# mkeeter/fidget

Measured on AMD Instinct MI355X. Metric: Mvoxel/s (interval+point eval) on prospero.vm 1024^3, higher is better.
Workload: dtype f32; 1 GPU; prospero.vm 3D heightmap+normals 1024^3, HipShape render hints (the library's tiles: 128/32/8, or 32/8 when the root level has few tiles), world_to_model=I

## Files before the change

### fidget_amd/csrc/capi_render.hpp

```cpp
static fhip_status bind_inputs(fhip_ctx* ctx, const fhip_tape* tape, const int32_t* axis_slots, const uint64_t* keys,
                               const float* vals, uint32_t n, FhRender& P) {
    const fh::HostTape& t = tape->t;
    std::vector<char> bound(FH_MAX_INPUTS, 0);
    for (uint32_t s = 0; s < FH_MAX_INPUTS; s++) { P.in_kind[s] = 3; P.in_value[s] = 0.0f; }
    for (int a = 0; a < 3; a++) {
        const int s = axis_slots ? axis_slots[a] : t.vars.axis[a];
        if (s >= 0 && s < FH_MAX_INPUTS) { P.in_kind[s] = (uint32_t)a; bound[s] = 1; }
    }
    for (uint32_t i = 0; i < n; i++) {
        const int s = axis_slots ? (int)keys[i] : t.vars.slot_of(3, keys[i]);
        if (s >= 0 && s < FH_MAX_INPUTS) { P.in_value[s] = vals[i]; bound[s] = 1; }
    }
    for (uint32_t s = 0; s < t.n_vars; s++)
        if (!bound[s]) return fail(ctx, FHIP_ERR_MISSING_VAR, "a variable of the shape has no value");
    return FHIP_OK;
}

struct HostSpans {
    double t[8] = {0, 0, 0, 0, 0, 0, 0, 0};
    uint64_t n = 0;
    std::chrono::steady_clock::time_point last;
    void start() { last = std::chrono::steady_clock::now(); }
    void mark(int k) { const auto now = std::chrono::steady_clock::now(); t[k] += std::chrono::duration<double, std::micro>(now - last).count(); last = now; }
    void frame() {
// ... 227 lines not shown
struct KaPrune1 { FhRenderState* S; uint32_t level, big, max_choices, mode; };
struct KaColumns { FhRenderState* S; uint32_t n_waves, slots, depmask, flags, pad[2]; const void* table; uint32_t nfpl, layers; };
struct KaNormals { FhRenderState* S; uint32_t n_waves, slots, z_lo, z_hi, bucket_cap, mode; };

struct FrameStreams { hipStream_t s[N_ROLES]; Role cur; hipStream_t on() const { return s[cur]; } };
static FrameStreams frame_streams(const fhip_ctx* ctx, Role at = CALLER) { return FrameStreams{{ctx->stream, ctx->stream_pre, ctx->stream2, ctx->stream3}, at}; }
static hipError_t hop(FrameStreams& fs, Role to, hipEvent_t ev) {
    if (to == fs.cur) return hipSuccess;
    const hipError_t e = hipEventRecord(ev, fs.on());
    fs.cur = to;
    return e != hipSuccess ? e : hipStreamWaitEvent(fs.on(), ev, 0);
}
static ScheduleInputs schedule_inputs(const fhip_ctx* ctx, int out_is_device) {
    ScheduleInputs in;
    in.no_tiles_v = ctx->opt.no_tiles_v; in.no_zrep = ctx->opt.no_zrep; in.column_walk = ctx->opt.column_walk; in.column_group = ctx->opt.column_group;
    in.frame_pipeline = ctx->frame_pipeline; in.use_pipeline = ctx->use_pipeline; in.profiling = ctx->profiling; in.slab_contexts = ctx->slab_contexts;
    in.has_side = ctx->stream2 != nullptr; in.has_tail = ctx->stream3 != nullptr; in.has_flags = ctx->host_flags != nullptr; in.out_is_device = out_is_device != 0;
    return in;
}
static char* rare_file(const fhip_ctx* ctx, const FhRenderState* dS, uint32_t rare_stride) {
    if (!rare_stride) return nullptr;
    return (char*)ctx->rare_scratch.p + (size_t)(dS - (const FhRenderState*)ctx->state.p) * FH_RARE_BLOCKS * rare_stride;
}
static void tiles_by_groups(fhip_ctx* ctx, const RenderSetup& R, FhRenderState* dS, hipStream_t st) {
    const int gg = blocks_for(ctx, R.lds_tiles_group, 8);
    KaTiles ka = {dS, 0, 1, R.group_regs, R.group_choices, (uint32_t)gg, (ctx->probe ? 1u : 0u) | 2u | 4u | 8u, 0, 0};
    (void)launch_asm(ctx, st, FH_ASM_TILES, (uint32_t)gg, &ka, sizeof(ka), R.lds_tiles_group);
    const uint32_t blocks = R.S.qcap[0], root_words = (R.S.troot_choices + 15) / 16, group_words = (R.group_choices + 15) / 16;
    if (R.S.top_chain && R.S.n_top > 64u * FH_CHAIN_SEG) FH_KLAUNCH(k_tchain3d_chunks, dim3(WAVE, blocks), dim3(WAVE), 0, st, dS);
    else if (R.S.top_chain) FH_KLAUNCH(k_tchain3d, dim3(WAVE, blocks), dim3(WAVE), 0, st, dS);
    else FH_KLAUNCH(k_ttop3d, dim3(blocks), dim3(WAVE), 0, st, dS);
    if (R.classify_only || !root_words) FH_KLAUNCH(k_tmark3d, dim3(blocks), dim3(WAVE), 0, st, dS);
    if (R.classify_only) return;
    if (root_words) FH_KLAUNCH(k_tscatter3d, dim3(root_words + 1, blocks), dim3(WAVE), 0, st, dS, group_words, root_words);
    KaPrune1 kp = {dS, 0, 1, R.S.troot_choices, 2};
    if (!R.prune2) { (void)launch_asm(ctx, st, FH_ASM_PRUNE1, blocks * 64, &kp, sizeof(kp)); return; }
    hipEvent_t ea = nullptr, eb = nullptr;
    if (ctx->profiling) { (void)hipEventCreate(&ea); (void)hipEventCreate(&eb); (void)hipEventRecord(ea, st); }
    FH_KLAUNCH(k_prune2, dim3(blocks * FH_P2_PER_SLOT), dim3(FH_P2_WPB * FH_P2_WPC * 64), R.lds_prune2, st, dS, 0u, 1u, root_words,
                       (const uint2*)R.d_links, (const uint2*)R.d_ctab, 2u, R.S.troot_len, R.S.troot_choices, R.p2_cap_kept,
                       (const uint32_t*)(R.d_ctab + std::max<uint32_t>(R.S.troot_choices, 1)), R.n_chain);
    size_t kp_bytes = sizeof(kp);
    void* extra[] = {HIP_LAUNCH_PARAM_BUFFER_POINTER, &kp, HIP_LAUNCH_PARAM_BUFFER_SIZE, &kp_bytes, HIP_LAUNCH_PARAM_END};
    (void)hipModuleLaunchKernel(ctx->asm_fn[FH_ASM_PRUNE1], blocks * 64, 1, 1, WAVE, 1, 1, 0, st, nullptr, extra);
    if (ctx->profiling) { (void)hipEventRecord(eb, st); ctx->asm_events.push_back({FH_ASM_PRUNE1, {ea, eb}}); }
}
static void tiles_asm(fhip_ctx* ctx, const RenderSetup& R, const LevelPlan& L, FhRenderState* dS, int level, FrameStreams& fs) {
    const int gs = blocks_for(ctx, R.lds_tiles_small, 8), gb = blocks_big(ctx, R, R.lds_tiles_big, 8);
    const int K_TILES = R.asm_tiles_t ? FH_ASM_TILES_T : FH_ASM_TILES;
    auto big_stream = [&] { return L.fork_big ? fs.s[SIDE] : fs.on(); };
    KaTiles ka = {dS, (uint32_t)level, 0, SMALL_REGS, SMALL_CHOICES, (uint32_t)gs, (ctx->probe ? 1u : 0u) | (L.exp ? 2u : 0u), 0, 0};
// ... 39 lines not shown
    if (R.full) FH_KLAUNCH((k_teval3d<true, true>), dim3(gb), dim3(WAVE), R.lds_tiles_big, st, dS, level);
    else FH_KLAUNCH((k_teval3d<false, true>), dim3(gb), dim3(WAVE), R.lds_tiles_big, st, dS, level);
}
static void launch_tiles_mono(fhip_ctx* ctx, const RenderSetup& R, FhRenderState* dS, int level, bool is3d, hipStream_t st) {
    const int gs = blocks_for(ctx, R.lds_tiles_small, 8), gb = blocks_big(ctx, R, R.lds_tiles_big, 8);
    launch(ctx, st, FHIP_K_TILES, [&] {
        if (is3d) { if (R.full) FH_LAUNCH_TILES(true, true, true, gb, R.lds_tiles_big); else FH_LAUNCH_TILES(true, false, true, gb, R.lds_tiles_big); }
        else { if (R.full) FH_LAUNCH_TILES(false, true, true, gb, R.lds_tiles_big); else FH_LAUNCH_TILES(false, false, true, gb, R.lds_tiles_big); }
    });
    if (level > 0)
        launch(ctx, st, FHIP_K_TILES, [&] {
            if (is3d) { if (R.full) FH_LAUNCH_TILES(true, true, false, gs, R.lds_tiles_small); else FH_LAUNCH_TILES(true, false, false, gs, R.lds_tiles_small); }
            else { if (R.full) FH_LAUNCH_TILES(false, true, false, gs, R.lds_tiles_small); else FH_LAUNCH_TILES(false, false, false, gs, R.lds_tiles_small); }
        });
}
static void launch_tiles(fhip_ctx* ctx, const RenderSetup& R, const LevelPlan& L, FhRenderState* dS, int level, bool is3d, FrameStreams& fs) {
    if (L.path == LevelPlan::MONO) return launch_tiles_mono(ctx, R, dS, level, is3d, fs.on());
    const int gp = ctx->n_cu * 8;
    launch(ctx, fs.on(), FHIP_K_TILES, [&] {
        if (is3d) FH_KLAUNCH(k_tsetup3d, dim3(gp), dim3(WAVE), 0, fs.on(), dS, level);
        else FH_KLAUNCH(k_tsetup2d, dim3(gp), dim3(WAVE), 0, fs.on(), dS, level);
    });
    launch(ctx, fs.on(), FHIP_K_TILES, [&] {
        if (L.path == LevelPlan::GROUPS) tiles_by_groups(ctx, R, dS, fs.on());
        else if (L.path == LevelPlan::ASM) tiles_asm(ctx, R, L, dS, level, fs);
        else tiles_hip(ctx, R, dS, level, fs.on());
    });
    const bool last = level + 1 == (int)R.S.P.n_levels;
    const int gpush = last ? ctx->n_cu * L.push_mul : gp;
    launch(ctx, fs.on(), FHIP_K_TILES, [&] {
        const uint32_t rb = L.rare ? FH_RARE_BLOCKS : 0u;
        if (is3d) FH_KLAUNCH(k_tpush3d, dim3(gpush + rb, last ? 1 : 17), dim3(WAVE), 0, fs.on(), dS, level, rb, rare_file(ctx, dS, L.rare_stride), L.rare_stride);
        else {
            if (!R.classify_only) FH_KLAUNCH(k_tpush2d, dim3(gpush), dim3(WAVE), 0, fs.on(), dS, level);
            const uint32_t slots_max = R.S.qcap[level] * ((level == 0 && R.groups) ? R.S.n_tgroups : 1u);
            FH_KLAUNCH(k_tfill2d, dim3(64, slots_max), dim3(256), 0, fs.on(), dS, level);
        }
    });
}

static fhip_status render2d_frame(fhip_ctx* ctx, const fhip_tape* tape, const fhip_render2d_config* cfg, float* out,
                                  int out_is_device) {
    if (ctx->is_cancelled()) return fail(ctx, FHIP_ERR_CANCELLED, "cancelled");
    RenderSetup R;
    memset(&R.S, 0, sizeof(R.S));
    FhRender& P = R.S.P;
    P.width = cfg->width; P.height = cfg->height; P.depth = 0; P.z = cfg->z; P.pixel_perfect = cfg->pixel_perfect ? 1 : 0;
// ... 528 lines not shown
```

### fidget_amd/csrc/frame_schedule.hpp

```cpp
#pragma once
#include <stddef.h>
#include <stdint.h>

#include <algorithm>
#include <vector>

#include "frame_plan.hpp"
#include "render_state.h"

static const uint32_t V32_REGS = 32, V32_CHOICES = 256, V64_REGS = 64, V64_CHOICES = 512;
static const uint32_t FH_RARE_BLOCKS = 8;

enum Role : uint8_t { CALLER = 0, PRE, SIDE, TAIL, N_ROLES };

struct ScheduleInputs {
    int no_tiles_v = 0, no_zrep = 0, column_walk = 1, column_group = 2;
    bool frame_pipeline = true, use_pipeline = true, profiling = false, has_side = true, has_tail = true, has_flags = true;
    uint32_t slab_contexts = 4;
    bool out_is_device = true, huge = false, whole = true;
    bool frames_queued = false;
    uint32_t pre_turn = 0;
    uint32_t rare_seen = 1, last_leaves = 0;
};

struct LevelPlan {
    enum Path : uint8_t { MONO, GROUPS, ASM, HIP } path = MONO;
    Role rest_on = CALLER;
    bool per_slab = false, exp = false;
    bool v32 = false, small_lds = false, v64 = false, both_lists = false;
    bool mid = false, rest = false;
    bool rare = false;
    bool fork_big = false;
    uint32_t rare_stride = 0; int push_mul = 2;
};

struct FrameSchedule {
    bool fpipe = false, lone = false, alt_pre = false, takes_turn = false;
    Role root = CALLER, l1_flags = CALLER, l1 = CALLER, fork_on = CALLER, tiles = CALLER, lists = CALLER, leaf = CALLER, normals = CALLER;
    bool fork_to_side = false, fork_to_tail = false, ev_pre = false, pre_implied = false, aux_edge = false;
    bool coarse = false, pipe = false, tiles_first = false; uint32_t NC = 1;
    int slab_first = 0, slab_stop = 0, n_rendered = 0;
    bool rare = false; uint32_t rare_stride = 0;
    enum LeafWalk : uint8_t { HIP_LEAVES, BY_LIST, BY_COLUMNS, BY_BLOCKS } leaf_walk = HIP_LEAVES;
    bool by_list = false, by_columns = false; uint32_t g = 0;
    uint32_t list_waves = 0, table_words = 0; int reset_blocks = 1;
    bool normals_on = true;
    LevelPlan level[FH_MAX_LEVELS];
};

static bool frame_pipelined(const ScheduleInputs& in) { return in.frame_pipeline && in.use_pipeline && !in.profiling && in.out_is_device && !in.huge; }

static LevelPlan plan_level(const RenderSetup& R, const ScheduleInputs& in, int level, bool is3d, uint32_t rare_stride, Role on, Role rest_on) {
    LevelPlan L;
#ifdef FH_PUSH_MUL
    L.push_mul = FH_PUSH_MUL;
#endif
    L.rare_stride = rare_stride; L.rest_on = rest_on;
    const uint32_t pre = R.S.pre_levels, l = (uint32_t)level;
    const FhRender& P = R.S.P;
    if (!R.split) return L;
    L.per_slab = pre > 0 && l >= pre;
    L.exp = R.prune1 && l < R.exp_levels;
    L.rare = rare_stride && is3d && R.asm_tiles && !in.no_tiles_v && level > 0 && L.per_slab && !L.exp;
    if (R.groups && level == 0) { L.path = LevelPlan::GROUPS; return L; }
    if (!R.asm_tiles) { L.path = LevelPlan::HIP; return L; }
    L.path = LevelPlan::ASM;
    L.fork_big = level > 0 && l < pre && in.use_pipeline && !in.profiling && in.has_side && on == CALLER && is3d;
    const bool vk = !in.no_tiles_v && !L.exp;
    L.both_lists = level > 0 && vk && l < pre && !L.fork_big;
    L.v32 = level > 0 && vk && !L.both_lists; L.small_lds = level > 0 && !vk;
    if (L.rare) return L;
    const bool root_v64 = vk && level == 0 && is3d && P.max_regs <= V64_REGS && P.max_choices <= V64_CHOICES;
    L.v64 = vk && (level > 0 || root_v64);
    L.rest = !L.v64 || P.max_regs > V64_REGS || P.max_choices > V64_CHOICES;
    L.mid = !vk && level > 0 && l < pre && R.lds_tiles_mid * 2 <= R.lds_tiles_big;
    return L;
}

static FrameSchedule schedule_frame(const RenderSetup& R, const ScheduleInputs& in) {
    FrameSchedule F;
    const FhRender& P = R.S.P;
    const uint32_t pre = R.S.pre_levels, n_groups = R.groups_per_slab, slabs = R.slab_hi - R.slab_lo;
    F.fpipe = frame_pipelined(in);
    F.alt_pre = F.fpipe && P.n_levels == 2 && R.column_inv && in.no_zrep == 0 && in.has_tail && in.whole;
    F.lone = F.fpipe && !in.frames_queued;
#ifdef FH_EXP_NO_LONE
    F.lone = false;
#endif
    F.takes_turn = F.fpipe && !F.lone && F.alt_pre;
    F.root = !F.fpipe || F.lone ? CALLER : (F.takes_turn && (in.pre_turn & 1u) ? TAIL : PRE);
    F.coarse = pre && n_groups;
    F.pipe = in.use_pipeline && !in.profiling && slabs > 1 && n_groups > 0 && !R.big_hbm;
    F.NC = F.pipe ? std::min<uint32_t>(in.slab_contexts, slabs) : 1;
    F.slab_first = (int)R.slab_hi - 1; F.slab_stop = (int)R.slab_stop;
    F.n_rendered = n_groups ? std::max(0, F.slab_first - F.slab_stop + 1) : 0;
    const bool l1_side = F.fpipe && !F.lone && pre > 1 && in.has_side && slabs > 1 && n_groups > 0;
    F.tiles_first = F.pipe && l1_side && R.root_invariant && in.has_tail && R.asm_points && slabs <= F.NC;
    F.l1 = l1_side ? SIDE : F.root;
    F.l1_flags = F.tiles_first ? F.root : F.l1;
    const bool tail_to_side = F.fpipe && !F.lone && F.pipe && pre == 1 && in.has_side;
    F.fork_on = F.tiles_first ? TAIL : tail_to_side ? SIDE : F.l1;
    F.tiles = !F.pipe ? CALLER : F.tiles_first ? TAIL : SIDE;
    F.fork_to_side = F.pipe && F.fork_on != SIDE;
    F.fork_to_tail = F.tiles_first;
    F.pre_implied = F.fpipe && F.pipe && pre == 1 && in.has_side && F.fork_on == SIDE;
    F.ev_pre = F.fpipe && F.fork_on != CALLER && !F.pre_implied;
    const bool on_main = F.tiles_first && in.frames_queued;
    F.aux_edge = F.pipe && in.has_tail && R.asm_points && !on_main && !F.alt_pre;
    F.lists = F.normals = F.aux_edge ? TAIL : CALLER;
    const size_t stride = (std::max(std::max(R.lds_tiles_big, R.lds_points_big), R.lds_normals_big) + 255) / 256 * 256;
    F.rare = R.split && R.asm_tiles && R.asm_points && R.asm_normals && !R.big_hbm && in.has_flags && in.rare_seen == 0 &&
             stride * FH_RARE_BLOCKS * 4 <= ((size_t)256 << 20);
    F.rare_stride = F.rare ? (uint32_t)stride : 0u;
    const uint32_t layers = P.slab / 8;
    F.by_list = in.column_walk == 1 && R.column_inv && R.split && R.zrep && R.asm_points && R.asm_normals && layers <= 64 && in.has_flags;
    F.table_words = F.by_list ? 0u : R.table_words;
    F.list_waves = (R.n_footprints + 63) / 64 * 64;
    if (F.by_list && in.last_leaves) F.list_waves = std::min(F.list_waves, (in.last_leaves + in.last_leaves / 8 + 63) / 64 * 64);
    F.reset_blocks = (int)std::max<uint32_t>(1, std::min<uint32_t>(1024, (std::max(F.table_words, n_groups) + 255) / 256));
    F.by_columns = in.column_walk == 2 || ((in.column_walk == 1 || in.column_walk == 3) && R.column_inv);
    const uint32_t g_opt = (uint32_t)std::min(std::max(in.column_group, 0), 6);
    F.g = F.by_columns ? 6u : (R.smooth_tape && g_opt > 1 ? g_opt - 1 : g_opt);
    F.leaf_walk = !R.asm_points ? FrameSchedule::HIP_LEAVES : F.by_list ? FrameSchedule::BY_LIST
// ... 11 lines not shown
```

### fidget_amd/csrc/gen_tilesv.py

```python
from gen_interp import OPS, UNSUPPORTED, HSTRIDE_LOG2
import gen_tiles as GT
from gen_tiles import (Tiles, S_KERNARG, S_STATE, S_LEVEL, S_BIG, S_MAXREGS, S_MAXCH, S_ARENA, S_ARENACAP, S_SLOTS, S_NSLOTS, S_SLOT, S_OFF,
                       S_LEN, S_RC, S_ACT, S_SIGN, S_ABSM, S_DECIDED, S_CI, S_NREGS, S_NCH, S_PRUNE, S_BASE, S_MA, S_MB, S_HBASE, S_TAPE,
                       S_REM, S_K, S_W0, S_W1, S_T0, S_OUT, S_A, S_T1, S_OP, S_RET, S_T64, S_LIVE, S_ALIAS, S_CIMM, S_KEEP, S_PC, S_SAVE,
                       S_M, S_T2, S_T3, S_SKIPR, S_SKIPC, S_SI, S_NWG, V_LANE, V_L4, VX, VY, VZ, AL, AH, BL, BH, RL, RH, T, V_CW, V_C,
                       V_RESL, V_RESH, V_QNAN, V_SQRTC, V_ONE, SLOT_SIZE, SL_ACT, SL_XYZ, SL_RES, SL_COFF, SL_CLEN, SL_CRC, TRANS_UNARY, T_SMAP)

SRC0, SRC1, SRC2, DST = 1, 2, 4, 8

S_CB = "s[48:49]"
S_N = "s50"
S_SENT = "s51"
S_PBASE = "s[52:53]"
S_JMP = "s[54:55]"
S_CHUNK = "s3"
S_OUTM = "s[56:57]"
S_ANYLIVE = "s[72:73]"
S_CBASE = "s17"
S_CWI = "s18"
HL = 9
S_M8 = "s[58:59]"
S_BIDX = "s60"
S_AEQB = "s61"

# ... 81 lines not shown
        self.a(f"\ts_set_gpr_idx_off\n\tv_mov_b32 {BL}, {S_W1}\n\tv_mov_b32 {BH}, {S_W1}")

    def imm_a_swap(self):
        self.a(f"""
	s_set_gpr_idx_off
	v_mov_b32 {BL}, {AL}
	v_mov_b32 {BH}, {AH}
	v_mov_b32 {AL}, {S_W1}
	v_mov_b32 {AH}, {S_W1}""")

    INLINE = {"abs", "square", "sqrt", "mul", "mulimm", "min", "max", "and", "or", "input"}

    def ool_body(self, stem, fn):
        if stem in self.INLINE:
            return fn()
        lab = f"{self.p}_b_{stem}"
        if not any(l == lab for l, _ in self.ool):
            self.ool.append((lab, fn))
        self.a(f"\ts_branch {lab}")

    def handler(self, op):
        a = self.a
        if op == "OUTPUT":
            a(f"\ts_set_gpr_idx_off\n\tv_mov_b32 {V_RESL}, {AL}\n\tv_mov_b32 {V_RESH}, {AH}")
            return self.dispatch()
        if op == "INPUT":
            a("\ts_set_gpr_idx_off")
            return self.ool_body("input", self.h_input)
        if op == "COPY_REG":
            a(f"\ts_set_gpr_idx_on {S_OUT}, {DST}\n\tv_pk_mov_b32 {self.F()}, v[10:11], v[10:11] op_sel:[0,1]")
            return self.dispatch()
        if op == "COPY_IMM":
            a(f"\ts_set_gpr_idx_off\n\tv_mov_b32 {RL}, {S_W1}\n\tv_mov_b32 {RH}, {S_W1}")
            return self.done()
        unary = {"NEG": self.b_neg, "ABS": self.b_abs, "RECIP": self.b_recip, "SQRT": self.b_sqrt, "SQUARE": self.b_square,
                 "NOT": self.b_not}
        if op in unary:
            def body(fn=unary[op]):
                fn()
                self.done()
            a("\ts_set_gpr_idx_off")
            if op == "NEG":
                return body()
            return self.ool_body(op.lower(), body)
        if op in TRANS_UNARY:
            def body(op=op):
                self.b_trans(op)
# ... 459 lines not shown
	s_and_b64 {S_MB}, {S_MB}, {S_LIVE}
	s_or_b64 {S_T64}, {S_MA}, {S_MB}
	s_andn2_b64 {S_SAVE}, {S_LIVE}, {S_T64}
	s_mov_b64 {S_ALIAS}, {S_MA}
	s_cmp_eq_u64 {S_ALIAS}, 0
	s_cbranch_scc1 {noalias}""")
        self.alias_path(S_MA, None)
        a(f"""
{noalias}:
	s_cmp_eq_u64 {S_MB}, 0
	s_cbranch_scc1 {nocimm}
	s_mov_b64 exec, {S_MB}""")
        self.pool_give(V_NO)
        self.ew0(3)
        a(f"\tv_mov_b32 {V_EW1}, {S_W1}")
        self.emit_op()
        a(f"""
{nocimm}:
	s_cmp_eq_u64 {S_SAVE}, 0
	s_cbranch_scc1 {p}_pnext
	s_mov_b64 exec, {S_SAVE}""")
        self.keep_path(S_SAVE, False, True)
        self.pnext()

    def emit_kernel(self):
        a, o, p, name = self.a, self.off, self.p, self.name
        a(f"""
	.text
	.protected {name}
	.globl {name}
	.p2align 8
	.type {name},@function
{name}:
	s_load_dwordx2 {S_STATE}, {S_KERNARG}, 0x0
	s_load_dwordx4 s[8:11], {S_KERNARG}, 0x8
	s_load_dwordx2 s[100:101], {S_KERNARG}, 0x18
	v_mov_b32 {V_QNAN}, 0x7fc00000
	v_mov_b32 {V_SQRTC}, 0xf800000
	v_mov_b32 {V_ONE}, 1
	v_mov_b32 {V_DEAD}, {DEADV}
	s_mov_b32 {S_SIGN}, 0x80000000
	s_mov_b32 {S_ABSM}, 0x7fffffff
	s_mov_b32 s58, -8
	s_mov_b32 s59, -1
	v_lshlrev_b32 {V_L8}, 3, {V_LANE}
	v_lshlrev_b32 {V_L4}, 2, {V_LANE}
# ... 88 lines not shown
	s_cbranch_scc1 {p}_outer
	s_memtime s[60:61]""")
        for k, r in enumerate((VX[0], VX[1], VY[0], VY[1], VZ[0], VZ[1])):
            a(f"\tglobal_load_dword {r}, {V_L4}, {S_SLOT} offset:{SL_XYZ + 256 * k}")
        a(f"""
	s_mov_b32 s44, {S_OFF}
	s_mov_b32 s45, 0
	s_lshl_b64 {S_TAPE}, {S_TAPE}, 3
	s_add_u32 s44, s44, s10
	s_addc_u32 s45, s45, s11
	s_mov_b32 {S_CI}, 0
	s_mov_b64 {S_DECIDED}, 0
""" + "".join(f"\tv_mov_b32 v{self.CHF + w}, 0\n" for w in range(self.ncw)) + f"""	v_mov_b32 {V_RESL}, {V_QNAN}
	v_mov_b32 {V_RESH}, {V_QNAN}
	s_getpc_b64 {S_RET}
{p}_pc1:
	s_add_u32 s74, s74, {p}_ret1 - {p}_pc1
	s_addc_u32 s75, s75, 0
	s_branch {p}_run
{p}_ret1:
	s_memtime s[62:63]
	global_store_dword {V_L4}, {V_RESL}, {S_SLOT} offset:{SL_RES}
	global_store_dword {V_L4}, {V_RESH}, {S_SLOT} offset:{SL_RES + 256}
	; ---- classify: ambiguous = act && !(hi < 0) && !(lo > 0); prune those whose trace decided something ------------
	v_cmp_gt_f32_e64 {S_M[0]}, 0, {V_RESH}
	v_cmp_gt_f32_e64 {S_M[1]}, {V_RESL}, 0
	v_mov_b32 {V_COFF}, {S_OFF}
	v_mov_b32 {V_CLEN}, {S_LEN}
	v_mov_b32 {V_CRC}, {S_RC}
	s_or_b64 {S_M[0]}, {S_M[0]}, {S_M[1]}
	s_andn2_b64 {S_PRUNE}, {S_ACT}, {S_M[0]}
	s_and_b64 {S_PRUNE}, {S_PRUNE}, {S_DECIDED}
	s_cmp_eq_u64 {S_PRUNE}, 0
	s_cbranch_scc1 {p}_store
	; ---- arena: every pruned child reserves a slot as long as the parent tape -------------------------------------------
	s_bcnt1_i32_b64 {S_T0}, {S_PRUNE}
	s_mul_i32 {S_T1}, {S_T0}, {S_LEN}
	v_mbcnt_lo_u32_b32 {V_RANK}, s34, 0
	v_mbcnt_hi_u32_b32 {V_RANK}, s35, {V_RANK}
	v_cmp_eq_u32 vcc, 0, {V_LANE}
	s_and_saveexec_b64 {S_SAVE}, vcc
	v_mov_b32 {T[0]}, {S_T1}
	v_mov_b32 {T[1]}, 0
	global_atomic_add {T[2]}, {T[1]}, {T[0]}, {S_STATE} offset:{o['arena_head']} sc0
	s_waitcnt vmcnt(0)
	s_mov_b64 exec, {S_SAVE}
# ... 12 lines not shown
	; in front of [choice table | links | tape] is frame_stamp << 32 | len | choices << 16 - is not pruned here: its choice words go
	; to chw[list] (16 words per slot in list 0, flags[31:16] in list 1), its ambiguous children are marked (c_len = ~0, c_off = the
	; end of their arena slot) and k_prune2, launched behind this kernel, writes their tapes - one wave per child instead of the
	; lockstep sweep over the parent's ops below.
	s_bitcmp1_b32 s101, 1
	s_cbranch_scc0 {p}_sweep
	s_add_u32 {S_T0}, {S_LEN}, {S_NCH}
	s_add_u32 {S_T0}, {S_T0}, 1
	s_sub_u32 s76, {S_OFF}, {S_T0}
	s_cbranch_scc1 {p}_sweep                          ; (the tape starts too low in the arena to have anything in front)
	s_mov_b32 s77, 0
	s_lshl_b64 s[76:77], s[76:77], 3
	s_add_u32 s76, s76, s10
	s_addc_u32 s77, s77, s11
	s_load_dwordx2 s[76:77], s[76:77], 0x0
	s_load_dword {S_T2}, {S_STATE}, {o['frame_stamp']}
	s_lshl_b32 {S_T1}, {S_NCH}, 16
	s_or_b32 {S_T1}, {S_T1}, {S_LEN}
	s_waitcnt lgkmcnt(0)
	s_cmp_eq_u32 s76, {S_T1}
	s_cbranch_scc0 {p}_sweep
	s_cmp_eq_u32 s77, {S_T2}
	s_cbranch_scc0 {p}_sweep
	; the choice words: chw[list] + slot index * stride
	s_bfe_u32 {S_T0}, s70, 0x10001                    ; which list
	s_lshl_b32 {S_T1}, {S_T0}, 3
	s_add_u32 s76, s4, {S_T1}
	s_addc_u32 s77, s5, 0
	s_load_dwordx2 s[76:77], s[76:77], {o['chw']}
	s_lshr_b32 {S_T2}, s101, 16
	s_cmp_eq_u32 {S_T0}, 0
	s_cselect_b32 {S_T2}, 16, {S_T2}
	s_lshl_b32 {S_T2}, {S_T2}, 8                      ; bytes per slot
	s_sub_u32 {S_T3}, {S_SI}, {S_NWG}                 ; this slot's index (the round robin has moved on)
	s_mul_hi_u32 {S_T1}, {S_T3}, {S_T2}
	s_mul_i32 {S_T3}, {S_T3}, {S_T2}
	s_waitcnt lgkmcnt(0)
	s_add_u32 s76, s76, {S_T3}
	s_addc_u32 s77, s77, {S_T1}
""" + "".join(("\ts_add_u32 s76, s76, 0x1000\n\ts_addc_u32 s77, s77, 0\n" if w and w % 16 == 0 else "") +
              f"\ts_cmp_le_u32 {S_NCH}, {16 * w}\n\ts_cbranch_scc1 {p}_exported\n\tglobal_store_dword {V_L4}, v{self.CHF + w}, s[76:77] offset:{(w % 16) * 256}\n"
              for w in range(self.ncw)) + f"""{p}_exported:
	v_mov_b32 {T[1]}, -1
	v_cndmask_b32_e64 {V_COFF}, {V_COFF}, {V_END}, {S_PRUNE}
	v_cndmask_b32_e64 {V_CLEN}, {V_CLEN}, {T[1]}, {S_PRUNE}
	s_branch {p}_store
{p}_sweep:
	v_mov_b32 {T[0]}, {V_END}
	v_mov_b32 {T[1]}, 0
	v_lshlrev_b64 {V_DST}, 3, v[16:17]
	v_mov_b32 {T[2]}, s11
	v_add_co_u32 v20, vcc, s10, v20
	s_nop 1
	v_addc_co_u32 v21, vcc, {T[2]}, v21, vcc
	s_getpc_b64 {S_RET}
{p}_pc2:
	s_add_u32 s74, s74, {p}_ret2 - {p}_pc2
	s_addc_u32 s75, s75, 0
	s_branch {p}_prune
{p}_ret2:
	s_mov_b64 exec, -1
	; child = {{ base + (rank + 1) * len - count, count, high | kept << 16 }} for the pruned lanes
	v_sub_u32 {V_END}, {V_END}, {V_COUNT}
	v_lshl_or_b32 {T[5]}, {V_KEPT}, 16, {V_HIGH}
	v_cndmask_b32_e64 {V_COFF}, {V_COFF}, {V_END}, {S_PRUNE}
	v_cndmask_b32_e64 {V_CLEN}, {V_CLEN}, {V_COUNT}, {S_PRUNE}
# ... 100 lines not shown
```

### fidget_amd/csrc/prune2.hip

```cpp
#pragma once
#include <hip/hip_runtime.h>

#include "render_state.h"

#define FH_P2_WPC 4
#define FH_P2_PER_SLOT ((64 + FH_P2_WPB - 1) / FH_P2_WPB)
enum { FH_LK_OUT = 0, FH_LK_NONE = 1, FH_LK_A = 2, FH_LK_RR = 3, FH_LK_COPY = 4, FH_LK_CRR = 5, FH_LK_CRI = 6 };
#define FH_LK_CHOICE 0x8000u
#define FH_LK_IMM 0x4000u

namespace fhp2 {
__device__ __forceinline__ uint32_t rfl(uint32_t v) { return __builtin_amdgcn_readfirstlane(v); }
__device__ __forceinline__ uint64_t rfl64(uint64_t v) { return (uint64_t)rfl((uint32_t)v) | ((uint64_t)rfl((uint32_t)(v >> 32)) << 32); }
__device__ __forceinline__ uint32_t excl_sum(uint32_t v, uint32_t lane, uint32_t& total) {
    uint32_t x = v;
#pragma unroll
    for (int d = 1; d < 64; d <<= 1) {
        const uint32_t y = __shfl_up(x, d, 64);
        if ((int)lane >= d) x += y;
    }
    total = __shfl(x, 63, 64);
    return x - v;
}
__device__ __forceinline__ void p2_scan_batch2(uint32_t u, uint32_t& rel, uint32_t& out, uint32_t& maxro, uint32_t cnt, uint32_t kabs0) {
#if defined(__HIP_DEVICE_COMPILE__)
    uint32_t k, su, ro, kabs = kabs0;
    asm volatile(
        "s_mov_b32 %[k], 0\n"
        "L_p2b_loop_%=:\n\t"
// ... 32 lines not shown
    const uint32_t sidx = blk / per_slot;
    const uint32_t G = rfl(S->n_tgroups);
    if (sidx * G >= rfl(S->n_slots[big][level])) return;
    FhSlot& sl = S->slots[big][(size_t)sidx * G];
    if (sl.act == 0) return;
    const uint32_t c0 = (blk % per_slot) * wpb, c = c0 + kid;
    {
        bool any = false;
        for (uint32_t k = 0; k < wpb; k++) any |= c0 + k < 64 && sl.c_len[c0 + k] == 0xFFFFFFFFu;
        if (!any) return;
    }
    const uint32_t off = rfl(sl.tape.off), n = rfl(sl.tape.len), nch = rfl((uint32_t)sl.tape.n_choices);
    if (n > cap_ops || nch > cap_choices) return;
    const uint2* const ops = (const uint2*)(S->arena + off);
    const uint2* const lks = links;
    uint32_t* const chl = (uint32_t*)(smem + (size_t)FH_P2_WPB * fh_p2_wave_lds(cap_choices, cap_kept));
    for (uint32_t i = threadIdx.x; i < n_chain; i += blockDim.x) chl[i] = chain[i];
    char* const mine = smem + (size_t)kid * fh_p2_wave_lds(cap_choices, cap_kept);
    uint64_t* const mask = (uint64_t*)mine;
    uint16_t* const pref = (uint16_t*)(mine + 1024);
    uint16_t* const E = (uint16_t*)(mine + 1280);
    uint2* const comp = (uint2*)(mine + 1280 + (((size_t)cap_choices * 2 + 15) & ~(size_t)15));
    uint32_t* const lastuse = (uint32_t*)((char*)comp + (size_t)cap_kept * 8);
    uint8_t* const regb = (uint8_t*)((char*)lastuse + (size_t)cap_kept * 4);
    uint32_t* const red = (uint32_t*)(regb + (size_t)cap_kept * 3);
    const uint32_t nw = (n + 63) >> 6;
    bool on = c < 64 && rfl(sl.c_len[min(c, 63u)]) == 0xFFFFFFFFu;
    if (on && tid < 4) red[tid] = 0;
    const uint32_t* const cws = S->chwr + (size_t)sidx * G * cw_stride * 64;
    uint32_t* const cwl = (uint32_t*)comp;
    if (on) for (uint32_t k = tid; k < (nch + 15) / 16; k += 64 * W) cwl[k] = cws[(size_t)k * 64 + c];
    __syncthreads();

    const bool probe = S->want_stats != 0 && (flags & 2u) != 0 && lead;
    const uint64_t t_a = probe ? clock64() : 0;
    if (on) {
        const uint32_t nb = (nch + 63) >> 6;
        uint2 tn = (sub * 64 + lane) < nch ? ctab[sub * 64 + lane] : make_uint2(0, 0);
        for (uint32_t bi = sub; bi < nb; bi += W) {
            const uint32_t q0 = bi << 6, q = q0 + lane;
            const uint2 t = tn;
            if (q + 64 * W < nch) tn = ctab[q + 64 * W];
            uint32_t e = 0;
            if (q < nch) {
                const uint32_t i = t.y & 0xFFFFu, kind = t.y >> 16;
                const uint32_t ch = (cwl[q >> 4] >> ((q & 15) * 2)) & 3u;
// ... 17 lines not shown
            const uint32_t e = q < nch ? (uint32_t)E[q] : 0u;
            const bool ptr = (e & FH_LK_CHOICE) != 0;
            if (__ballot(ptr) == 0) continue;
            if (ptr) E[q] = E[e & 0x7FFFu];
        }
    }
    __syncthreads();
    auto resolve = [&](uint2 l, bool& has_a, bool& has_b, bool& imm, uint32_t& ta, uint32_t& tb) {
        const uint32_t kind = (l.x >> 8) & 0xFFu, fa = l.y & 0xFFFFu, fb = l.y >> 16;
        const uint32_t e_own = E[kind == FH_LK_CRI ? (l.x >> 16) : 0u];
        const uint32_t e_a = E[((fa & FH_LK_CHOICE) && fa != 0xFFFFu) ? (fa & 0x7FFFu) : 0u], e_b = E[((fb & FH_LK_CHOICE) && fb != 0xFFFFu) ? (fb & 0x7FFFu) : 0u];
        imm = kind == FH_LK_CRI && (e_own & FH_LK_IMM) != 0;
        has_a = !imm && kind != FH_LK_NONE;
        has_b = !imm && (kind == FH_LK_RR || kind == FH_LK_CRR);
        ta = (fa & FH_LK_CHOICE) ? (e_a & 0x3FFFu) : fa;
        tb = (fb & FH_LK_CHOICE) ? (e_b & 0x3FFFu) : fb;
    };

    const uint64_t t_b1 = probe ? clock64() : 0;
    if (on && lead) {
        for (uint32_t k = lane; k < 128; k += 64) mask[k] = (k == ((n - 1) >> 6)) ? 1ull << ((n - 1) & 63) : 0ull;
        const uint32_t cw_bytes = (((nch + 15) / 16) * 4 + 15) & ~15u;
        uint16_t* const queue = (uint16_t*)((char*)comp + cw_bytes);
        const uint32_t qcap = (cap_kept * 8u - cw_bytes) / 2u;
        if (lane == 0) queue[0] = (uint16_t)(n - 1);
        uint32_t head = 0, tail = 1;
        bool over = false;
        const uint64_t below = (1ull << lane) - 1;
        for (uint32_t top = n_chain; top > 0;) {
            const uint32_t cnt = min(64u, top);
            uint32_t ch = 0, i = 0;
            if (lane < cnt) {
                const uint32_t e = chl[top - 1 - lane], q = e & 0xFFFFu;
                i = e >> 16;
                ch = (cwl[q >> 4] >> ((q & 15) * 2)) & 3u;
            }
            const uint64_t cut = __ballot(ch == FH_CHOICE_RIGHT);
            const bool seed = ch == FH_CHOICE_BOTH && (cut == 0 || lane < (uint32_t)__builtin_ctzll(cut));
            if (seed) atomicOr((unsigned long long*)&mask[i >> 6], 1ull << (i & 63));
            const uint64_t ms = __ballot(seed);
            if (tail + (uint32_t)__popcll(ms) > qcap) { over = true; break; }
            if (seed) queue[tail + (uint32_t)__popcll(ms & below)] = (uint16_t)i;
            tail += (uint32_t)__popcll(ms);
            if (cut) break;
            top -= cnt;
        }
        while (!over && head < tail) {
            const uint32_t cnt = min(64u, tail - head);
            bool has_a = false, has_b = false, imm = false;
            uint32_t ta = 0, tb = 0;
            if (lane < cnt) resolve(lks[queue[head + lane]], has_a, has_b, imm, ta, tb);
            head += cnt;
            bool new_a = false, new_b = false;
            if (has_a) { const uint64_t bit = 1ull << (ta & 63); new_a = (atomicOr((unsigned long long*)&mask[ta >> 6], bit) & bit) == 0; }
            if (has_b) { const uint64_t bit = 1ull << (tb & 63); new_b = (atomicOr((unsigned long long*)&mask[tb >> 6], bit) & bit) == 0; }
            const uint64_t ma = __ballot(new_a), mb = __ballot(new_b);
            const uint32_t na = (uint32_t)__popcll(ma), nb = (uint32_t)__popcll(mb);
            if (tail + na + nb > qcap) { over = true; break; }
            if (new_a) queue[tail + (uint32_t)__popcll(ma & below)] = (uint16_t)ta;
            if (new_b) queue[tail + na + (uint32_t)__popcll(mb & below)] = (uint16_t)tb;
            tail += na + nb;
        }
        if (over && lane == 0) red[3] = 1;
    }
    if (on && lead) {
        const uint32_t k0 = lane < nw ? (uint32_t)__popcll(mask[lane]) : 0u, k1 = lane + 64 < nw ? (uint32_t)__popcll(mask[lane + 64]) : 0u;
        uint32_t t0, t1;
        const uint32_t e0 = excl_sum(k0, lane, t0), e1 = excl_sum(k1, lane, t1);
        pref[lane] = (uint16_t)e0; pref[lane + 64] = (uint16_t)(t0 + e1);
        if (lane == 0) { red[0] = t0 + t1; if (t0 + t1 > cap_kept) red[3] = 1; }
    }
    __syncthreads();
    const uint64_t t_b2 = probe ? clock64() : 0;
    const uint32_t m = on ? rfl(red[0]) : 0u;
    if (on && rfl(red[3]) != 0) {
        if (probe && lane == 0) atomicAdd(&S->leaf_stat[5], 1ull << 32);
        on = false;
    }
    if (on) for (uint32_t k = tid; k < m; k += 64 * W) lastuse[k] = 0;
    __syncthreads();
    auto pos_of = [&](uint32_t t) -> uint32_t { return (uint32_t)pref[t >> 6] + (uint32_t)__popcll(mask[t >> 6] & ((1ull << (t & 63)) - 1)); };
    if (on) {
        for (uint32_t b = sub; b < nw; b += W) {
            const uint64_t word = rfl64(mask[b]);
            if (word == 0) continue;
            if ((word >> lane) & 1) {
                const uint32_t i = (b << 6) | lane;
                const uint32_t p = (uint32_t)pref[b] + (uint32_t)__popcll(word & ((1ull << lane) - 1));
                const uint2 l = lks[i];
                bool has_a, has_b, imm;
                uint32_t ta, tb;
                resolve(l, has_a, has_b, imm, ta, tb);
                const uint32_t kind = (l.x >> 8) & 0xFFu;
                uint32_t pa = 0, pb = 0;
                if (has_a) { pa = pos_of(ta); atomicMax(&lastuse[pa], p); }
                if (has_b) { pb = pos_of(tb); atomicMax(&lastuse[pb], p); }
                const uint32_t fl = (has_a ? 1u : 0u) | (has_b ? 2u : 0u) | (imm ? 4u : 0u) | ((kind >= FH_LK_CRR && !imm) ? 8u : 0u) | (kind == FH_LK_OUT ? 16u : 0u);
                comp[p] = make_uint2(pa | (pb << 16), i | (fl << 16));
            }
        }
    }
    __syncthreads();
    const uint64_t t_b3 = probe ? clock64() : 0;
    if (on && lead) {
        uint32_t maxro = 0, rel = 0;
        for (uint32_t base = 0; base < m; base += 64) {
            const uint32_t pl = base + lane;
            const uint32_t u = pl < m ? lastuse[pl] : 0u;
            uint32_t outv = 0;
            p2_scan_batch2(u, rel, outv, maxro, min(64u, m - base), base);
            if (pl < m) regb[pl] = (uint8_t)outv;
        }
        if (maxro >= 64u) {
            if (probe && lane == 0) { atomicAdd(&S->leaf_stat[4], 1ull << 32); atomicMax(&S->leaf_stat[6], (unsigned long long)m << 32); }
            if (lane == 0) red[3] = 1;
        }
    }
    __syncthreads();
    if (on && rfl(red[3]) != 0) on = false;
    const uint32_t end = on ? rfl(sl.c_off[c]) : 0u;
    if (on) {
        uint64_t* const dst = S->arena + (end - m);
// ... 34 lines not shown
```

Baseline: 9.796 million Mvoxel/s.

## Add forward-only v64 group-tiles path and cache resolved links in prune2

At the root level with term groups, the planner can now pick a v64 assembly tiles kernel whose new flag bit stops after the forward pass. That pass exports the results, the term intervals (written in the OUTPUT handler) and the choice words, and skips classification, the arena and pruning. The shared choice-word export code is moved into a helper. In prune2, the BFS records each queued node's resolved operands and flags in a packed word, so the compaction phase reads those records instead of rescanning the mask and re-resolving links. This caps the queue at five rounds of waves, and it relies on 13-bit operand indices and on the new kernel variant being present and correct.

```diff
diff --git a/fidget_amd/csrc/capi_render.hpp b/fidget_amd/csrc/capi_render.hpp
--- a/fidget_amd/csrc/capi_render.hpp
+++ b/fidget_amd/csrc/capi_render.hpp
@@ -273,11 +273,16 @@
     if (!rare_stride) return nullptr;
     return (char*)ctx->rare_scratch.p + (size_t)(dS - (const FhRenderState*)ctx->state.p) * FH_RARE_BLOCKS * rare_stride;
 }
-static void tiles_by_groups(fhip_ctx* ctx, const RenderSetup& R, FhRenderState* dS, hipStream_t st) {
+static void tiles_by_groups(fhip_ctx* ctx, const RenderSetup& R, const LevelPlan& L, FhRenderState* dS, hipStream_t st) {
     const int gg = blocks_for(ctx, R.lds_tiles_group, 8);
+    const uint32_t blocks = R.S.qcap[0], root_words = (R.S.troot_choices + 15) / 16, group_words = (R.group_choices + 15) / 16;
     KaTiles ka = {dS, 0, 1, R.group_regs, R.group_choices, (uint32_t)gg, (ctx->probe ? 1u : 0u) | 2u | 4u | 8u, 0, 0};
-    (void)launch_asm(ctx, st, FH_ASM_TILES, (uint32_t)gg, &ka, sizeof(ka), R.lds_tiles_group);
-    const uint32_t blocks = R.S.qcap[0], root_words = (R.S.troot_choices + 15) / 16, group_words = (R.group_choices + 15) / 16;
+    if (L.groups_v64) {
+        ka.n_waves = (uint32_t)(ctx->n_cu * 8);
+        ka.flags |= group_words << 16;
+        (void)launch_asm(ctx, st, FH_ASM_TILES_V64, ka.n_waves, &ka, sizeof(ka));
+    } else
+        (void)launch_asm(ctx, st, FH_ASM_TILES, (uint32_t)gg, &ka, sizeof(ka), R.lds_tiles_group);
     if (R.S.top_chain && R.S.n_top > 64u * FH_CHAIN_SEG) FH_KLAUNCH(k_tchain3d_chunks, dim3(WAVE, blocks), dim3(WAVE), 0, st, dS);
     else if (R.S.top_chain) FH_KLAUNCH(k_tchain3d, dim3(WAVE, blocks), dim3(WAVE), 0, st, dS);
     else FH_KLAUNCH(k_ttop3d, dim3(blocks), dim3(WAVE), 0, st, dS);
@@ -363,7 +368,7 @@
         else FH_KLAUNCH(k_tsetup2d, dim3(gp), dim3(WAVE), 0, fs.on(), dS, level);
     });
     launch(ctx, fs.on(), FHIP_K_TILES, [&] {
-        if (L.path == LevelPlan::GROUPS) tiles_by_groups(ctx, R, dS, fs.on());
+        if (L.path == LevelPlan::GROUPS) tiles_by_groups(ctx, R, L, dS, fs.on());
         else if (L.path == LevelPlan::ASM) tiles_asm(ctx, R, L, dS, level, fs);
         else tiles_hip(ctx, R, dS, level, fs.on());
     });
diff --git a/fidget_amd/csrc/frame_schedule.hpp b/fidget_amd/csrc/frame_schedule.hpp
--- a/fidget_amd/csrc/frame_schedule.hpp
+++ b/fidget_amd/csrc/frame_schedule.hpp
@@ -29,6 +29,7 @@
     bool per_slab = false, exp = false;
     bool v32 = false, small_lds = false, v64 = false, both_lists = false;
     bool mid = false, rest = false;
+    bool groups_v64 = false;
     bool rare = false;
     bool fork_big = false;
     uint32_t rare_stride = 0; int push_mul = 2;
@@ -62,7 +63,11 @@
     L.per_slab = pre > 0 && l >= pre;
     L.exp = R.prune1 && l < R.exp_levels;
     L.rare = rare_stride && is3d && R.asm_tiles && !in.no_tiles_v && level > 0 && L.per_slab && !L.exp;
-    if (R.groups && level == 0) { L.path = LevelPlan::GROUPS; return L; }
+    if (R.groups && level == 0) {
+        L.path = LevelPlan::GROUPS;
+        L.groups_v64 = !in.no_tiles_v && R.group_regs <= V64_REGS && R.group_choices <= V64_CHOICES;
+        return L;
+    }
     if (!R.asm_tiles) { L.path = LevelPlan::HIP; return L; }
     L.path = LevelPlan::ASM;
     L.fork_big = level > 0 && l < pre && in.use_pipeline && !in.profiling && in.has_side && on == CALLER && is3d;
@@ -98,7 +103,11 @@
     F.tiles_first = F.pipe && l1_side && R.root_invariant && in.has_tail && R.asm_points && slabs <= F.NC;
     F.l1 = l1_side ? SIDE : F.root;
     F.l1_flags = F.tiles_first ? F.root : F.l1;
+#ifdef FH_EXP_FORK_ON_ROOT
+    const bool tail_to_side = false;
+#else
     const bool tail_to_side = F.fpipe && !F.lone && F.pipe && pre == 1 && in.has_side;
+#endif
     F.fork_on = F.tiles_first ? TAIL : tail_to_side ? SIDE : F.l1;
     F.tiles = !F.pipe ? CALLER : F.tiles_first ? TAIL : SIDE;
     F.fork_to_side = F.pipe && F.fork_on != SIDE;
diff --git a/fidget_amd/csrc/gen_tilesv.py b/fidget_amd/csrc/gen_tilesv.py
--- a/fidget_amd/csrc/gen_tilesv.py
+++ b/fidget_amd/csrc/gen_tilesv.py
@@ -127,7 +127,19 @@
     def handler(self, op):
         a = self.a
         if op == "OUTPUT":
-            a(f"\ts_set_gpr_idx_off\n\tv_mov_b32 {V_RESL}, {AL}\n\tv_mov_b32 {V_RESH}, {AH}")
+            skip = self.lab("out")
+            a(f"""
+	s_set_gpr_idx_off
+	v_mov_b32 {V_RESL}, {AL}
+	v_mov_b32 {V_RESH}, {AH}
+	s_bitcmp1_b32 s101, 3
+	s_cbranch_scc0 {skip}
+	s_load_dwordx2 s[76:77], {S_SLOT}, 0x20
+	s_lshl_b32 {S_T1}, {S_W1}, 9
+	v_add_u32 {T[0]}, {S_T1}, {V_L8}
+	s_waitcnt lgkmcnt(0)
+	global_store_dwordx2 {T[0]}, v[34:35], s[76:77]
+{skip}:""")
             return self.dispatch()
         if op == "INPUT":
             a("\ts_set_gpr_idx_off")
@@ -633,6 +645,28 @@
 	s_mov_b64 exec, {S_SAVE}""")
         self.keep_path(S_SAVE, False, True)
         self.pnext()
+
+    def export_text(self, done):
+        o = self.off
+        return f"""	; the choice words: chw[list] + slot index * stride
+	s_bfe_u32 {S_T0}, s70, 0x10001                    ; which list
+	s_lshl_b32 {S_T1}, {S_T0}, 3
+	s_add_u32 s76, s4, {S_T1}
+	s_addc_u32 s77, s5, 0
+	s_load_dwordx2 s[76:77], s[76:77], {o['chw']}
+	s_lshr_b32 {S_T2}, s101, 16
+	s_cmp_eq_u32 {S_T0}, 0
+	s_cselect_b32 {S_T2}, 16, {S_T2}
+	s_lshl_b32 {S_T2}, {S_T2}, 8                      ; bytes per slot
+	s_sub_u32 {S_T3}, {S_SI}, {S_NWG}                 ; this slot's index (the round robin has moved on)
+	s_mul_hi_u32 {S_T1}, {S_T3}, {S_T2}
+	s_mul_i32 {S_T3}, {S_T3}, {S_T2}
+	s_waitcnt lgkmcnt(0)
+	s_add_u32 s76, s76, {S_T3}
+	s_addc_u32 s77, s77, {S_T1}
+""" + "".join(("\ts_add_u32 s76, s76, 0x1000\n\ts_addc_u32 s77, s77, 0\n" if w and w % 16 == 0 else "") +
+              f"\ts_cmp_le_u32 {S_NCH}, {16 * w}\n\ts_cbranch_scc1 {done}\n\tglobal_store_dword {V_L4}, v{self.CHF + w}, s[76:77] offset:{(w % 16) * 256}\n"
+              for w in range(self.ncw)) + f"{done}:\n"
 
     def emit_kernel(self):
         a, o, p, name = self.a, self.off, self.p, self.name
@@ -767,6 +801,12 @@
 	s_memtime s[62:63]
 	global_store_dword {V_L4}, {V_RESL}, {S_SLOT} offset:{SL_RES}
 	global_store_dword {V_L4}, {V_RESH}, {S_SLOT} offset:{SL_RES + 256}
+	; flags bit 2 (the root level's term groups, as in fh_tiles): the forward pass only - the results above, the terms' intervals
+	; (bit 3, the OUTPUT handler) and the slot's choice words, laid out as fh_tiles exports them; no classification, no arena, no prune
+	s_bitcmp1_b32 s101, 2
+	s_cbranch_scc0 {p}_classify
+""" + self.export_text(f"{p}_gexported") + f"""	s_branch {p}_outer
+{p}_classify:
 	; ---- classify: ambiguous = act && !(hi < 0) && !(lo > 0); prune those whose trace decided something ------------
 	v_cmp_gt_f32_e64 {S_M[0]}, 0, {V_RESH}
 	v_cmp_gt_f32_e64 {S_M[1]}, {V_RESL}, 0
@@ -825,26 +865,7 @@
 	s_cbranch_scc0 {p}_sweep
 	s_cmp_eq_u32 s77, {S_T2}
 	s_cbranch_scc0 {p}_sweep
-	; the choice words: chw[list] + slot index * stride
-	s_bfe_u32 {S_T0}, s70, 0x10001                    ; which list
-	s_lshl_b32 {S_T1}, {S_T0}, 3
-	s_add_u32 s76, s4, {S_T1}
-	s_addc_u32 s77, s5, 0
-	s_load_dwordx2 s[76:77], s[76:77], {o['chw']}
-	s_lshr_b32 {S_T2}, s101, 16
-	s_cmp_eq_u32 {S_T0}, 0
-	s_cselect_b32 {S_T2}, 16, {S_T2}
-	s_lshl_b32 {S_T2}, {S_T2}, 8                      ; bytes per slot
-	s_sub_u32 {S_T3}, {S_SI}, {S_NWG}                 ; this slot's index (the round robin has moved on)
-	s_mul_hi_u32 {S_T1}, {S_T3}, {S_T2}
-	s_mul_i32 {S_T3}, {S_T3}, {S_T2}
-	s_waitcnt lgkmcnt(0)
-	s_add_u32 s76, s76, {S_T3}
-	s_addc_u32 s77, s77, {S_T1}
-""" + "".join(("\ts_add_u32 s76, s76, 0x1000\n\ts_addc_u32 s77, s77, 0\n" if w and w % 16 == 0 else "") +
-              f"\ts_cmp_le_u32 {S_NCH}, {16 * w}\n\ts_cbranch_scc1 {p}_exported\n\tglobal_store_dword {V_L4}, v{self.CHF + w}, s[76:77] offset:{(w % 16) * 256}\n"
-              for w in range(self.ncw)) + f"""{p}_exported:
-	v_mov_b32 {T[1]}, -1
+""" + self.export_text(f"{p}_exported") + f"""	v_mov_b32 {T[1]}, -1
 	v_cndmask_b32_e64 {V_COFF}, {V_COFF}, {V_END}, {S_PRUNE}
 	v_cndmask_b32_e64 {V_CLEN}, {V_CLEN}, {T[1]}, {S_PRUNE}
 	s_branch {p}_store
diff --git a/fidget_amd/csrc/prune2.hip b/fidget_amd/csrc/prune2.hip
--- a/fidget_amd/csrc/prune2.hip
+++ b/fidget_amd/csrc/prune2.hip
@@ -5,6 +5,8 @@
 
 #define FH_P2_WPC 4
 #define FH_P2_PER_SLOT ((64 + FH_P2_WPB - 1) / FH_P2_WPB)
+#define FH_P2_REC_ROUNDS 5
+static_assert(FH_P2_REC_ROUNDS * 64 * FH_P2_WPC >= FH_P2_MAX_KEPT, "B2 takes a child's records in FH_P2_REC_ROUNDS rounds of its waves");
 enum { FH_LK_OUT = 0, FH_LK_NONE = 1, FH_LK_A = 2, FH_LK_RR = 3, FH_LK_COPY = 4, FH_LK_CRR = 5, FH_LK_CRI = 6 };
 #define FH_LK_CHOICE 0x8000u
 #define FH_LK_IMM 0x4000u
@@ -83,6 +85,7 @@
     uint16_t* const E = (uint16_t*)(mine + 1280);
     uint2* const comp = (uint2*)(mine + 1280 + (((size_t)cap_choices * 2 + 15) & ~(size_t)15));
     uint32_t* const lastuse = (uint32_t*)((char*)comp + (size_t)cap_kept * 8);
+    uint32_t* const rec = lastuse;
     uint8_t* const regb = (uint8_t*)((char*)lastuse + (size_t)cap_kept * 4);
     uint32_t* const red = (uint32_t*)(regb + (size_t)cap_kept * 3);
     const uint32_t nw = (n + 63) >> 6;
@@ -146,7 +149,7 @@
         for (uint32_t k = lane; k < 128; k += 64) mask[k] = (k == ((n - 1) >> 6)) ? 1ull << ((n - 1) & 63) : 0ull;
         const uint32_t cw_bytes = (((nch + 15) / 16) * 4 + 15) & ~15u;
         uint16_t* const queue = (uint16_t*)((char*)comp + cw_bytes);
-        const uint32_t qcap = (cap_kept * 8u - cw_bytes) / 2u;
+        const uint32_t qcap = min(min((cap_kept * 8u - cw_bytes) / 2u, cap_kept), (uint32_t)FH_P2_REC_ROUNDS * 64u * W);
         if (lane == 0) queue[0] = (uint16_t)(n - 1);
         uint32_t head = 0, tail = 1;
         bool over = false;
@@ -173,7 +176,13 @@
             const uint32_t cnt = min(64u, tail - head);
             bool has_a = false, has_b = false, imm = false;
             uint32_t ta = 0, tb = 0;
-            if (lane < cnt) resolve(lks[queue[head + lane]], has_a, has_b, imm, ta, tb);
+            if (lane < cnt) {
+                const uint2 l = lks[queue[head + lane]];
+                resolve(l, has_a, has_b, imm, ta, tb);
+                const uint32_t kind = (l.x >> 8) & 0xFFu;
+                const uint32_t fl = (has_a ? 1u : 0u) | (has_b ? 2u : 0u) | (imm ? 4u : 0u) | ((kind >= FH_LK_CRR && !imm) ? 8u : 0u) | (kind == FH_LK_OUT ? 16u : 0u);
+                rec[head + lane] = (ta & 0x1FFFu) | ((tb & 0x1FFFu) << 13) | (fl << 26);
+            }
             head += cnt;
             bool new_a = false, new_b = false;
             if (has_a) { const uint64_t bit = 1ull << (ta & 63); new_a = (atomicOr((unsigned long long*)&mask[ta >> 6], bit) & bit) == 0; }
@@ -201,27 +210,27 @@
         if (probe && lane == 0) atomicAdd(&S->leaf_stat[5], 1ull << 32);
         on = false;
     }
-    if (on) for (uint32_t k = tid; k < m; k += 64 * W) lastuse[k] = 0;
+    uint32_t ri[FH_P2_REC_ROUNDS], rw[FH_P2_REC_ROUNDS];
+    {
+        const uint16_t* const queue = (const uint16_t*)((const char*)comp + ((((nch + 15) / 16) * 4 + 15) & ~15u));
+#pragma unroll
+        for (int j = 0; j < FH_P2_REC_ROUNDS; j++) {
+            const uint32_t k = tid + (uint32_t)j * 64u * W;
+            ri[j] = 0; rw[j] = 0;
+            if (on && k < m) { ri[j] = queue[k]; rw[j] = rec[k]; lastuse[k] = 0; }
+        }
+    }
     __syncthreads();
     auto pos_of = [&](uint32_t t) -> uint32_t { return (uint32_t)pref[t >> 6] + (uint32_t)__popcll(mask[t >> 6] & ((1ull << (t & 63)) - 1)); };
-    if (on) {
-        for (uint32_t b = sub; b < nw; b += W) {
-            const uint64_t word = rfl64(mask[b]);
-            if (word == 0) continue;
-            if ((word >> lane) & 1) {
-                const uint32_t i = (b << 6) | lane;
-                const uint32_t p = (uint32_t)pref[b] + (uint32_t)__popcll(word & ((1ull << lane) - 1));
-                const uint2 l = lks[i];
-                bool has_a, has_b, imm;
-                uint32_t ta, tb;
-                resolve(l, has_a, has_b, imm, ta, tb);
-                const uint32_t kind = (l.x >> 8) & 0xFFu;
-                uint32_t pa = 0, pb = 0;
-                if (has_a) { pa = pos_of(ta); atomicMax(&lastuse[pa], p); }
-                if (has_b) { pb = pos_of(tb); atomicMax(&lastuse[pb], p); }
-                const uint32_t fl = (has_a ? 1u : 0u) | (has_b ? 2u : 0u) | (imm ? 4u : 0u) | ((kind >= FH_LK_CRR && !imm) ? 8u : 0u) | (kind == FH_LK_OUT ? 16u : 0u);
-                comp[p] = make_uint2(pa | (pb << 16), i | (fl << 16));
-            }
+#pragma unroll
+    for (int j = 0; j < FH_P2_REC_ROUNDS; j++) {
+        if (on && tid + (uint32_t)j * 64u * W < m) {
+            const uint32_t i = ri[j], ta = rw[j] & 0x1FFFu, tb = (rw[j] >> 13) & 0x1FFFu, fl = rw[j] >> 26;
+            const uint32_t p = pos_of(i);
+            uint32_t pa = 0, pb = 0;
+            if (fl & 1u) { pa = pos_of(ta); atomicMax(&lastuse[pa], p); }
+            if (fl & 2u) { pb = pos_of(tb); atomicMax(&lastuse[pb], p); }
+            comp[p] = make_uint2(pa | (pb << 16), i | (fl << 16));
         }
     }
     __syncthreads();
```

After: 9.529 million Mvoxel/s. 0.973x the previous value.
